# lorenzrichter/path-space-PDE-solver

Hardware: AMD Instinct MI355X
Metric: trajectory-timesteps/sec (K*N/s), d=100 HJB log-variance training iteration (higher is better)
Workload: dtype f32 (f16x3 split products: every matrix product as three f16 MFMAs, fp32 accumulate; state / sums fp32)

## Files before the change

### path-space-pde-solver_amd/csrc/hjb_kernels.h

```cpp
#pragma once
#include <cstdlib>
#include <type_traits>
#include <hip/hip_runtime.h>
#include <stdint.h>

namespace psp {

typedef float f32x4 __attribute__((ext_vector_type(4)));

struct HjbArgs {
    const float* params;
    const float* x0;
    const float* y0;
    const float* xi;
    float* path;
    float* D;
    float* XN;
    double* fwd_partial;
    const float* drift;
    const float* sigma;
    const float* runcost;
    const float* term;
    const double* sums;
    float* grad_partial;
// ... 95 lines not shown
    return p + opaque_i(0);
}

#define PSP_PATH_STORE(ptr, val) __builtin_nontemporal_store((val), (ptr))

#ifndef PSP_PHILOX_ROUNDS
#define PSP_PHILOX_ROUNDS 7
#endif
constexpr int kPhiloxRounds = PSP_PHILOX_ROUNDS;
__device__ __forceinline__ void philox4x32_R(uint32_t c0, uint32_t c1, uint32_t c2, uint32_t c3,
                                             uint32_t k0, uint32_t k1, uint32_t (&out)[4]) {
#pragma unroll
    for (int r = 0; r < kPhiloxRounds; ++r) {
        const unsigned long long p0 = (unsigned long long)0xD2511F53u * (unsigned long long)c0;
        const unsigned long long p1 = (unsigned long long)0xCD9E8D57u * (unsigned long long)c2;
        const uint32_t hi0 = (uint32_t)(p0 >> 32), lo0 = (uint32_t)p0;
        const uint32_t hi1 = (uint32_t)(p1 >> 32), lo1 = (uint32_t)p1;
        const uint32_t n0 = __builtin_amdgcn_bitop3_b32(hi1, c1, k0, 0x96), n2 = __builtin_amdgcn_bitop3_b32(hi0, c3, k1, 0x96);
        c0 = n0; c1 = lo1; c2 = n2; c3 = lo0;
        k0 += 0x9E3779B9u; k1 += 0xBB67AE85u;
    }
    out[0] = c0; out[1] = c1; out[2] = c2; out[3] = c3;
}

__device__ __forceinline__ void philox_round(uint32_t& c0, uint32_t& c1, uint32_t& c2, uint32_t& c3, uint32_t k0, uint32_t k1) {
    const unsigned long long p0 = (unsigned long long)0xD2511F53u * (unsigned long long)c0;
    const unsigned long long p1 = (unsigned long long)0xCD9E8D57u * (unsigned long long)c2;
    const uint32_t hi0 = (uint32_t)(p0 >> 32), lo0 = (uint32_t)p0;
    const uint32_t hi1 = (uint32_t)(p1 >> 32), lo1 = (uint32_t)p1;
    const uint32_t n0 = __builtin_amdgcn_bitop3_b32(hi1, c1, k0, 0x96), n2 = __builtin_amdgcn_bitop3_b32(hi0, c3, k1, 0x96);
    c0 = n0; c1 = lo1; c2 = n2; c3 = lo0;
}

__device__ __forceinline__ f32x4 normal4(const uint32_t (&r)[4]) {
    const float s24 = 1.0f / 16777216.0f, h24 = 0.5f / 16777216.0f;
    const float u0 = __builtin_fmaf((float)(r[0] >> 8), s24, h24);
    const float u1 = __builtin_fmaf((float)(r[1] >> 8), s24, h24);
    const float u2 = __builtin_fmaf((float)(r[2] >> 8), s24, h24);
    const float u3 = __builtin_fmaf((float)(r[3] >> 8), s24, h24);
    const float ra = __builtin_amdgcn_sqrtf(-1.3862943611198906f * __builtin_amdgcn_logf(u0));
    const float rb = __builtin_amdgcn_sqrtf(-1.3862943611198906f * __builtin_amdgcn_logf(u2));
    f32x4 z;
    z[0] = ra * __builtin_amdgcn_cosf(u1);
    z[1] = ra * __builtin_amdgcn_sinf(u1);
    z[2] = rb * __builtin_amdgcn_cosf(u3);
    z[3] = rb * __builtin_amdgcn_sinf(u3);
    return z;
}

__device__ __forceinline__ f32x4 philox_block(uint32_t kglob, uint32_t step, uint32_t idx, uint32_t iter,
                                              uint32_t seed_lo, uint32_t seed_hi) {
    uint32_t r[4];
    philox4x32_R(kglob, step, idx, iter, seed_lo, seed_hi, r);
    return normal4(r);
}

template <int D, int DB>
__device__ __forceinline__ void regen_xi(f32x4 (&xin)[DB], uint32_t kglob, uint32_t n, int q, uint32_t iter,
                                         uint32_t seed_lo, uint32_t seed_hi) {
#pragma unroll
    for (int b = 0; b < DB; ++b) {
        xin[b] = philox_block(kglob, n, (uint32_t)(4 * b + q), iter, seed_lo, seed_hi);
        if (16 * b + 16 > D) {
#pragma unroll
            for (int r = 0; r < 4; ++r) if (16 * b + 4 * r + q >= D) xin[b][r] = 0.f;
        }
    }
}

template <class F>
__device__ __forceinline__ void stage_aop(float* dst, int MB, int KS, int tid, int nthr, F src) {
    const int total = MB * KS * 64;
    for (int idx = tid; idx < total; idx += nthr) {
        const int lane = idx & 63, t = idx >> 6;
        const int ks = t % KS, mb = t / KS;
        const int i = lane & 15, q = lane >> 4;
        dst[idx] = src(16 * mb + 4 * (i & 3) + (i >> 2), 4 * ks + q);
    }
}
template <class F>
__device__ __forceinline__ void stage_vec(float* dst, int NBLK, int tid, int nthr, F v) {
    for (int idx = tid; idx < NBLK * 16; idx += nthr) {
        const int r = idx & 3, q = (idx >> 2) & 3, b = idx >> 4;
        dst[idx] = v(16 * b + 4 * r + q);
    }
}
// ... 456 lines not shown
    __syncthreads();

    const int t16 = blockIdx.x * nwave + wave;
    const bool wave_valid = t16 < a.ntile16;
    const int k = t16 * 16 + j;
    const bool kvalid = wave_valid && k < a.K_local;
    const uint32_t kglob = (uint32_t)(a.k_offset + k);
    const float dt = a.dt, sqdt = a.sqdt;

    const float store_cxi = SPEC ? 1.f : ((k_store == 3) ? 0.f : 1.f);
    const float store_cz = SPEC ? 0.f : ((k_store == 3) ? 1.f : (k_store == 2 ? -a.sqdt : (k_adaptive ? 0.f : a.sqdt)));
    const bool do_store = FAST ? true : (k_store != 0);
    double sD = 0.0, sD2 = 0.0;
    if (wave_valid) {
        const f32x4* vecs0 = reinterpret_cast<const f32x4*>(lds + VEC) + q;
        const f32x4* vterm = vecs0 + (G::vterm - G::fVec) / 4;

        f32x4 X[DB];
#pragma unroll
        for (int b = 0; b < DB; ++b) {
#pragma unroll
            for (int r = 0; r < 4; ++r) {
                const int f = 16 * b + 4 * r + q;
                const float v = a.x0[(size_t)(kvalid ? k : 0) * a.x0_stride + (f < D ? f : D - 1)];
                X[b][r] = (f < D && kvalid) ? v : 0.f;
            }
        }
        float Y = a.y0 ? a.y0[0] : 0.f;
        float Fsum = 0.f, ULsum = 0.f;
#ifdef PSP_STAMPS
        unsigned long long stamps[8] = {0, 0, 0, 0, 0, 0, 0, 0};
#endif

        for (int n = 0; n < a.N; ++n) {
            PSP_STAMP(fs0);
            float tn = (float)n * dt;
            if constexpr (!FAST) { if (a.tfeat) tn = a.tfeat[n]; }
            const f32x4* vecs = opaque(vecs0);
            const f32x4* vb1 = vecs + (G::vb1 - G::fVec) / 4;
            const f32x4* vw1t = vecs + (G::vw1t - G::fVec) / 4;
            const f32x4* vb2 = vecs + (G::vb2 - G::fVec) / 4;
            const f32x4* vb3 = vecs + (G::vb3 - G::fVec) / 4;
            const f32x4* vdr = vecs + (G::vdr - G::fVec) / 4;
            const f32x4* vrun = vecs + (G::vrun - G::fVec) / 4;
            float* pblk = a.path + ((size_t)n * a.ntile16 + t16) * (size_t)G::PB + lane;
            auto x_store = [&](int u, int NU) __attribute__((always_inline)) {
                if (do_store) {
#pragma unroll
                    for (int ks = 0; ks < 4 * DB; ++ks)
                        if (ks >= u * (4 * DB) / NU && ks < (u + 1) * (4 * DB) / NU)
                            PSP_PATH_STORE(pblk + (G::pX / 64 + ks) * 64, X[ks >> 2][ks & 3]);
                }
            };
            if (!X3 && do_store) {
#pragma unroll
                for (int ks = 0; ks < 4 * DB; ++ks) PSP_PATH_STORE(pblk + (G::pX / 64 + ks) * 64, X[ks >> 2][ks & 3]);
            }
            f32x4 h1[HB];
#pragma unroll
            for (int m = 0; m < HB; ++m) h1[m] = vb1[m * 4] + tn * vw1t[m * 4];
            f32x4 Tn[DB];
            const bool early_drift = X3 && k_drift == DRIFT_DENSE;
            if constexpr (X3) {
                if (k_drift == DRIFT_DENSE) {
                    f16x8 xh[DB / 2 > 0 ? DB / 2 : 1], xl[DB / 2 > 0 ? DB / 2 : 1];
                    constexpr int NU1 = (DB / 2) * HB, NU2 = (DB / 2) * DB;
                    split_panel8<DB>(X, xh, xl);
                    gemm_Txs<HB, KSD, DB, 2>(h1, lds + oW1, xh, xl, X[DB - 1], lane, [&](int u) __attribute__((always_inline)) { x_store(u, NU1 + NU2); });
#pragma unroll
                    for (int b = 0; b < DB; ++b) Tn[b] = X[b];
                    gemm_Txs<DB, KSD, DB, 2>(Tn, ldsA, xh, xl, X[DB - 1], lane, [&](int u) __attribute__((always_inline)) { x_store(NU1 + u, NU1 + NU2); });
                    if constexpr (NU1 + NU2 == 0) x_store(0, 1);
                } else {
                    constexpr int NU1 = (DB / 2) * HB;
                    gemm_Tx<HB, KSD, DB, 2>(h1, lds + oW1, X, lane, [&](int u) __attribute__((always_inline)) { x_store(u, NU1); });
                    if constexpr (NU1 == 0) x_store(0, 1);
                }
            }
            else if constexpr (BF16) gemm_Tb<HB, DB>(h1, lds + oW1, X, lane);
            else gemm_T<HB, KSD, DB>(h1, lds + oW1, X, lane);
            PSP_STAMP(fs1);
#pragma unroll
            for (int m = 0; m < HB; ++m) h1[m] = tanh4(h1[m]);
            PSP_STAMP(fs2);
            f32x4 h2[HB];
#pragma unroll
            for (int m = 0; m < HB; ++m) h2[m] = vb2[m * 4];
            constexpr int NUH2 = (HB / 2) * HB, NUH3 = (HB / 2) * DB;
            constexpr bool PREGEN = X3 && FAST && (NUH2 + NUH3 > 0);
            [[maybe_unused]] f32x4 xig[PREGEN ? DB : 1];
            [[maybe_unused]] uint32_t pc0 = 0, pc1 = 0, pc2 = 0, pc3 = 0;
            constexpr int NSPC = kPhiloxRounds + 1;
            auto philox_slice = [&](int sidx) __attribute__((always_inline)) {
                const int b = sidx / NSPC, sub = sidx % NSPC;
                if (sub == 0) { pc0 = kglob; pc1 = (uint32_t)n; pc2 = (uint32_t)(4 * b + q); pc3 = iter_now; }
                if (sub < kPhiloxRounds) {
                    philox_round(pc0, pc1, pc2, pc3, a.seed_lo + (uint32_t)sub * 0x9E3779B9u, a.seed_hi + (uint32_t)sub * 0xBB67AE85u);
                    asm volatile("" : "+v"(pc0), "+v"(pc1), "+v"(pc2), "+v"(pc3));
                } else {
                    const uint32_t rr[4] = {pc0, pc1, pc2, pc3};
                    f32x4 xi = normal4(rr);
                    if (16 * b + 16 > D) {
#pragma unroll
                        for (int r = 0; r < 4; ++r) if (16 * b + 4 * r + q >= D) xi[r] = 0.f;
                    }
                    asm volatile("" : "+v"(xi));
                    xig[b < DB ? b : 0] = xi;
                }
            };
            auto philox_portion = [&](int u) __attribute__((always_inline)) {
                if constexpr (PREGEN) {
#pragma unroll
                    for (int sidx = 0; sidx < NSPC * DB; ++sidx)
                        if (sidx >= u * (NSPC * DB) / (NUH2 + NUH3) && sidx < (u + 1) * (NSPC * DB) / (NUH2 + NUH3)) philox_slice(sidx);
                }
            };
            auto h_store = [&](const f32x4 (&h)[HB], int slot, int u, int NU) __attribute__((always_inline)) {
                if (do_store) {
#pragma unroll
                    for (int ks = 0; ks < 4 * HB; ++ks)
                        if (ks >= u * (4 * HB) / NU && ks < (u + 1) * (4 * HB) / NU)
                            PSP_PATH_STORE(pblk + (slot / 64 + ks) * 64, h[ks >> 2][ks & 3]);
                }
            };
            if constexpr (X3) {
                gemm_Tx<HB, KSH, HB, 2>(h2, lds + oW2, h1, lane, [&](int u) __attribute__((always_inline)) { h_store(h1, G::pH1, u, NUH2); philox_portion(u); });
                if constexpr (NUH2 == 0) h_store(h1, G::pH1, 0, 1);
            }
            else if constexpr (BF16) gemm_Tb<HB, HB>(h2, lds + oW2, h1, lane);
            else gemm_T<HB, KSH, HB>(h2, lds + oW2, h1, lane);
// ... 615 lines not shown
```

### path-space-pde-solver_amd/csrc/hjbx_kernels.h

```cpp
#pragma once
#include "hjb_kernels.h"

namespace psp {

template <int D, int H>
struct GeoX {
    using G = Geo<D, H>;
    static constexpr int DB = G::DB, HB = G::HB, KSD = G::KSD, KSH = G::KSH;
    static constexpr int T3 = 0, T2 = T3 + SplitGeo<KSD, DB>::floats(HB), EX = T2 + SplitGeo<KSH, HB>::floats(HB);
    static constexpr int hG = 0, hGl = hG + D * 32, hZ2 = hGl + D * 32, hZ2l = hZ2 + HB * 512, hZ1 = hZ2l + HB * 512,
                         hZ1l = hZ1 + HB * 512, PAIRH = hZ1l + HB * 512;
    static constexpr int RS = 16 * DB + 3 * 16 * HB;
    static constexpr int NX = cdiv(DB, 4);
    static constexpr int NT = DB + 2 * HB;
    static_assert(4 * RS <= 4 * (PAIRH / 2), "bias sums reuse the exchange area");
    static constexpr int GS = EX + 4 * (PAIRH / 2);
    static int lds_floats() { return GS + 12; }
};

template <int NB>
__device__ __forceinline__ void split_panel(const f32x4 (&v)[NB], f16x4 (&hi)[NB], f16x4 (&lo)[NB]) {
#pragma unroll
    for (int b = 0; b < NB; ++b) {
        if ((NB & 1) && b == NB - 1) split4c(v[b], hi[b], lo[b]);
        else split4(v[b], hi[b], lo[b]);
    }
}

template <int MB, int KS, int INB>
__device__ __forceinline__ void gemm_Txp(f32x4 (&acc)[MB], const float* wlds, const f16x4 (&hi)[INB], const f16x4 (&lo)[INB],
                                         float last, int lane) {
    using SG = SplitGeo<KS, INB>;
    constexpr int NS = SG::NS;
    lane = opaque_i(lane);
    f32x4 corr[MB];
#pragma unroll
    for (int mb = 0; mb < MB; ++mb) corr[mb] = f32x4{0.f, 0.f, 0.f, 0.f};
    if constexpr (NS > 0) {
        const f16x8* tbl = reinterpret_cast<const f16x8*>(wlds) + lane;
        constexpr int NU = NS * MB, CU = 1, NCH = cdiv(NU, CU);
        f16x8 ah[2][CU], al[2][CU];
#pragma unroll
        for (int kk = 0; kk < CU; ++kk)
            if (kk < NU) {
                ah[0][kk] = tbl[((kk % MB) * SG::per_mb + (kk / MB) * 512) / 4];
                al[0][kk] = tbl[((kk % MB) * SG::per_mb + (kk / MB) * 512) / 4 + 64];
            }
#pragma unroll
// ... 17 lines not shown
                    const f16x8 bl = __builtin_shufflevector(lo[2 * S], lo[2 * S + 1], 0, 1, 2, 3, 4, 5, 6, 7);
                    acc[mb] = __builtin_amdgcn_mfma_f32_16x16x32_f16(ah[c & 1][kk], bh, acc[mb], 0, 0, 0);
                    corr[mb] = __builtin_amdgcn_mfma_f32_16x16x32_f16(ah[c & 1][kk], bl, corr[mb], 0, 0, 0);
                    corr[mb] = __builtin_amdgcn_mfma_f32_16x16x32_f16(al[c & 1][kk], bh, corr[mb], 0, 0, 0);
                }
            }
            __builtin_amdgcn_sched_barrier(kFenceMask);
        }
    }
    if constexpr (SG::ODD_F32) {
#pragma unroll
        for (int mb = 0; mb < MB; ++mb) acc[mb] = mfma16(wlds[mb * SG::per_mb + NS * 512 + lane], last, acc[mb]);
    }
    if constexpr (SG::ODD_H16) {
#pragma unroll
        for (int mb = 0; mb < MB; ++mb) {
            const f16x4* p = reinterpret_cast<const f16x4*>(wlds + mb * SG::per_mb + NS * 512) + lane;
            const f16x4 a_hi = p[0], a_lo = p[64];
            acc[mb] = __builtin_amdgcn_mfma_f32_16x16x16f16(a_hi, hi[INB - 1], acc[mb], 0, 0, 0);
            corr[mb] = __builtin_amdgcn_mfma_f32_16x16x16f16(a_hi, lo[INB - 1], corr[mb], 0, 0, 0);
            corr[mb] = __builtin_amdgcn_mfma_f32_16x16x16f16(a_lo, hi[INB - 1], corr[mb], 0, 0, 0);
        }
    }
#pragma unroll
    for (int mb = 0; mb < MB; ++mb) acc[mb] = acc[mb] + kSplitInv * corr[mb];
}

template <int D, int H, bool REGEN = false>
__global__ __launch_bounds__(512) void hjb_bwd3_kernel(const HjbArgs a) {
    PSP_COND_EXIT(a);
    GradCheck<true> gchk;
    using G = Geo<D, H>;
    using X = GeoX<D, H>;
    constexpr int DB = G::DB, HB = G::HB, KSD = G::KSD, KSH = G::KSH, NX = X::NX, RS = X::RS, PAIRH = X::PAIRH, NT = X::NT;
    extern __shared__ __attribute__((aligned(16))) float lds[];
    const int tid = threadIdx.x, nthr = blockDim.x;
    const int lane = tid & 63, wave = __builtin_amdgcn_readfirstlane(tid >> 6);
    const int j = lane & 15, q = lane >> 4;
    const bool producer = wave < 4;
    const int sub = wave & 3;
    const float* __restrict__ P = a.params;

    const double invK = 1.0 / (double)a.K_global;
    const float meanD = (a.loss_kind == LOSS_LOGVAR) ? (float)(a.sums[0] * invK) : 0.f;
    const float coef = (float)(2.0 * invK);
    {
        float wm = 0.f;
        for (int k = tid; k < a.K_local; k += nthr) {
            const float dk = a.D[k];
            wm = fmaxf(wm, fabsf(a.loss_kind == LOSS_WEIGHTS ? dk : coef * (dk - meanD)));
        }
#pragma unroll
        for (int o = 1; o < 64; o <<= 1) wm = fmaxf(wm, __shfl_xor(wm, o));
        if (lane == 0) lds[X::GS + 4 + wave] = wm;
    }
    stage_aop_x3<KSD, DB>(lds + X::T3, HB, tid, nthr, [&](int row, int col) {
        return (row < H && col < D) ? P[G::oW3 + col * H + row] : 0.f; });
    stage_aop_x3<KSH, HB>(lds + X::T2, HB, tid, nthr, [&](int row, int col) {
        return (row < H && col < H) ? P[G::oW2 + col * H + row] : 0.f; });
    __syncthreads();
    _Float16* exh = reinterpret_cast<_Float16*>(lds + X::EX);
    const bool xi_image = a.adaptive != 0 && (a.store_path == 1 || a.store_path == 4);
    auto g_scale = [&](float& gs, float& ginv) __attribute__((always_inline)) {
        const float* slot = lds + X::GS;
        float imax = fmaxf(fmaxf(slot[0], slot[1]), fmaxf(slot[2], slot[3]));
        if (xi_image || !(imax >= 1.1754944e-38f)) imax = xi_image ? 8.0f : 1.0f;
        const float wmax = fmaxf(fmaxf(fmaxf(slot[4], slot[5]), fmaxf(slot[6], slot[7])),
                                 fmaxf(fmaxf(slot[8], slot[9]), fmaxf(slot[10], slot[11])));
        const float amax = wmax * a.sqdt * imax;
        const unsigned e = (__float_as_uint(amax) >> 23) & 0xFFu;
        const bool ok = e >= 1u && e <= 253u;
        gs = ok ? __uint_as_float((254u - e) << 23) : 1.0f;
        ginv = ok ? __uint_as_float(e << 23) : 1.0f;
    };
    const f32x4 zero4 = {0.f, 0.f, 0.f, 0.f};
    const float sqdt = a.sqdt, dt = a.dt;
    constexpr bool regen = REGEN;
    const uint32_t iter_now = a.iter_dev ? *a.iter_dev : a.iter;
    const long long nblk = (long long)a.N * a.ntile16;
    const long long nround = (nblk + 3) / 4;
    const int R = (int)((nround - blockIdx.x + gridDim.x - 1) / gridDim.x);

    if (producer) {
        f32x4 sG[DB], sZ2[HB], sZ1[HB], sT1[HB];
#pragma unroll
        for (int b = 0; b < DB; ++b) sG[b] = zero4;
#pragma unroll
        for (int m = 0; m < HB; ++m) { sZ2[m] = zero4; sZ1[m] = zero4; sT1[m] = zero4; }
        auto own_block = [&](int it2) __attribute__((always_inline)) {
            const long long b0 = ((long long)blockIdx.x + (long long)it2 * gridDim.x) * 4 + sub;
            return b0 < nblk ? b0 : -1LL;
        };
        auto path_of = [&](int it2) __attribute__((always_inline)) {
            const long long b0 = own_block(it2);
            return a.path + (size_t)(b0 >= 0 ? b0 : nblk - 1) * (size_t)G::PB + lane;
        };
        f32x4 xin[DB], h2n[HB], h1n[HB];
        float dkn;
        {
            const long long b0 = own_block(0);
            const long long blk = b0 >= 0 ? b0 : nblk - 1;
            const float* pb = path_of(0);
            const int k0 = (int)(blk % a.ntile16) * 16 + j;
            dkn = a.D[k0 < a.K_local ? k0 : 0];
            if constexpr (regen) {
#pragma unroll
                for (int b = 0; b < DB; ++b) xin[b] = zero4;
            } else {
#pragma unroll
                for (int b = 0; b < DB; ++b)
#pragma unroll
                    for (int r = 0; r < 4; ++r) xin[b][r] = pb[G::pXi + (4 * b + r) * 64];
            }
            if constexpr (regen) {
#pragma unroll
                for (int m = 0; m < HB; ++m)
#pragma unroll
                    for (int r = 0; r < 4; ++r) h2n[m][r] = pb[G::pH2 + (4 * m + r) * 64];
#pragma unroll
                for (int m = 0; m < HB; ++m)
#pragma unroll
                    for (int r = 0; r < 4; ++r) h1n[m][r] = pb[G::pH1 + (4 * m + r) * 64];
            }
        }
        float gs, ginv;
        {
            const long long b0 = own_block(0);
            const int k0 = (int)((b0 >= 0 ? b0 : nblk - 1) % a.ntile16) * 16 + j;
            const bool kv = b0 >= 0 && k0 < a.K_local;
            float am = 0.f;
#pragma unroll
            for (int b = 0; b < DB; ++b)
#pragma unroll
                for (int r = 0; r < 4; ++r) am = fmaxf(am, kv ? fabsf(xin[b][r]) : 0.f);
#pragma unroll
            for (int o = 1; o < 64; o <<= 1) am = fmaxf(am, __shfl_xor(am, o));
            if (lane == 0) lds[X::GS + sub] = am;
            __syncthreads();
            g_scale(gs, ginv);
        }
#ifdef PSP_STAMPS
        unsigned long long stamps[8] = {0, 0, 0, 0, 0, 0, 0, 0};
#endif
        for (int it = 0; it <= R; ++it) {
            PSP_STAMP(tp0);
            if (it < R) {
                const long long blk0 = own_block(it);
                const bool bvalid = blk0 >= 0;
                const long long blk = bvalid ? blk0 : nblk - 1;
                const int t16 = (int)(blk % a.ntile16);
                const int k = t16 * 16 + j;
                const bool kvalid = bvalid && k < a.K_local;
                const float tn = (float)(blk / a.ntile16) * dt;
                _Float16* ex0 = exh + ((it & 1) * 2 + (sub >> 1)) * PAIRH + (sub & 1) * 4 + (j & 3);
                _Float16* exr[4] = {ex0 + (((j >> 2) ^ 0) * 8), ex0 + (((j >> 2) ^ 1) * 8), ex0 + (((j >> 2) ^ 2) * 8), ex0 + (((j >> 2) ^ 3) * 8)};
                const float* pn = path_of(it + 1);
                const float* pc = path_of(it);
                const float dkc = dkn;
                if constexpr (!regen) {
#pragma unroll
                    for (int m = 0; m < HB; ++m)
#pragma unroll
                        for (int r = 0; r < 4; ++r) h2n[m][r] = pc[G::pH2 + (4 * m + r) * 64];
                }
                const float wk = kvalid ? (a.loss_kind == LOSS_WEIGHTS ? dkc : coef * (dkc - meanD)) : 0.f;
                f32x4 Gt[DB];
                if constexpr (regen) {
                    const uint32_t kg = (uint32_t)(a.k_offset + k), nstep = (uint32_t)(blk / a.ntile16);
                    const int qo = opaque_i(q);
#pragma unroll
                    for (int b = 0; b < DB; ++b) {
                        f32x4 xi = philox_block(kg, nstep, (uint32_t)(4 * b + qo), iter_now, a.seed_lo, a.seed_hi);
                        if (16 * b + 16 > D) {
#pragma unroll
                            for (int r = 0; r < 4; ++r) if (16 * b + 4 * r + q >= D) xi[r] = 0.f;
                        }
                        {
#pragma clang fp contract(off)
                            Gt[b] = (wk * sqdt * gs) * xi;
                            sG[b] += Gt[b];
                        }
                        __builtin_amdgcn_sched_barrier(0);
                    }
                } else {
                    {
#pragma clang fp contract(off)
#pragma unroll
                        for (int b = 0; b < DB; ++b) {
                            Gt[b] = (wk * sqdt * gs) * xin[b];
                            sG[b] += Gt[b];
                        }
                    }
                }
                PSP_STAMP(tp1);
                PSP_ACC(0, tp1, tp0);
                f16x4 Gh[DB], Gl[DB];
                split_panel<DB>(Gt, Gh, Gl);
#pragma unroll
                for (int b = 0; b < DB; ++b)
#pragma unroll
                    for (int r = 0; r < 4; ++r) {
                        const int f = 16 * b + 4 * r + q;
                        if (16 * b + 16 <= D || f < D) {
                            exr[r][X::hG + f * 32] = Gh[b][r];
                            exr[r][X::hGl + f * 32] = Gl[b][r];
                        }
                    }
                PSP_STAMP(tp2);
                PSP_ACC(1, tp2, tp1);
                f32x4 dz2[HB];
#pragma unroll
                for (int m = 0; m < HB; ++m) dz2[m] = zero4;
                gemm_Txp<HB, KSD, DB>(dz2, lds + X::T3, Gh, Gl, Gt[DB - 1][0], lane);
                {
#pragma clang fp contract(off)
#pragma unroll
                    for (int m = 0; m < HB; ++m) { dz2[m] = dz2[m] * (1.0f - h2n[m] * h2n[m]); sZ2[m] += dz2[m]; }
                }
                if constexpr (regen) {
                    __builtin_amdgcn_sched_barrier(0);
#pragma unroll
                    for (int m = 0; m < HB; ++m)
#pragma unroll
                        for (int r = 0; r < 4; ++r) h2n[m][r] = pn[G::pH2 + (4 * m + r) * 64];
                } else {
#pragma unroll
                    for (int m = 0; m < HB; ++m)
#pragma unroll
                        for (int r = 0; r < 4; ++r) h1n[m][r] = pc[G::pH1 + (4 * m + r) * 64];
                    const long long n0 = own_block(it + 1);
                    const long long nb1 = n0 >= 0 ? n0 : nblk - 1;
                    const int k1 = (int)(nb1 % a.ntile16) * 16 + j;
                    dkn = a.D[k1 < a.K_local ? k1 : 0];
#pragma unroll
                    for (int b = 0; b < DB; ++b)
#pragma unroll
                        for (int r = 0; r < 4; ++r) xin[b][r] = pn[G::pXi + (4 * b + r) * 64];
                }
                PSP_STAMP(tp3);
                PSP_ACC(2, tp3, tp2);
                f16x4 Zh[HB], Zl[HB];
                split_panel<HB>(dz2, Zh, Zl);
#pragma unroll
                for (int m = 0; m < HB; ++m)
#pragma unroll
                    for (int r = 0; r < 4; ++r) {
                        exr[r][X::hZ2 + (16 * m + 4 * r + q) * 32] = Zh[m][r];
                        exr[r][X::hZ2l + (16 * m + 4 * r + q) * 32] = Zl[m][r];
                    }
                f32x4 dz1[HB];
#pragma unroll
                for (int m = 0; m < HB; ++m) dz1[m] = zero4;
                gemm_Txp<HB, KSH, HB>(dz1, lds + X::T2, Zh, Zl, dz2[HB - 1][0], lane);
                {
#pragma clang fp contract(off)
#pragma unroll
                    for (int m = 0; m < HB; ++m) {
                        dz1[m] = dz1[m] * (1.0f - h1n[m] * h1n[m]);
                        sZ1[m] += dz1[m];
                        sT1[m] += tn * dz1[m];
                    }
                }
                if constexpr (regen) {
                    __builtin_amdgcn_sched_barrier(0);
                    const long long n0 = own_block(it + 1);
                    const long long nb1 = n0 >= 0 ? n0 : nblk - 1;
                    const int k1 = (int)(nb1 % a.ntile16) * 16 + j;
                    dkn = a.D[k1 < a.K_local ? k1 : 0];
#pragma unroll
                    for (int m = 0; m < HB; ++m)
#pragma unroll
                        for (int r = 0; r < 4; ++r) h1n[m][r] = pn[G::pH1 + (4 * m + r) * 64];
                }
                split_panel<HB>(dz1, Zh, Zl);
#pragma unroll
                for (int m = 0; m < HB; ++m)
#pragma unroll
                    for (int r = 0; r < 4; ++r) {
                        exr[r][X::hZ1 + (16 * m + 4 * r + q) * 32] = Zh[m][r];
                        exr[r][X::hZ1l + (16 * m + 4 * r + q) * 32] = Zl[m][r];
                    }
            }
            PSP_STAMP(tp4);
            PSP_ACC(3, tp4, tp0);
            __syncthreads();
            PSP_STAMP(tp5);
            PSP_ACC(4, tp5, tp4);
            PSP_ACC(6, tp5, tp0);
        }
#ifdef PSP_STAMPS
        if (a.dbg && lane == 0) {
            stamps[7] = (unsigned long long)R;
            for (int i = 0; i < 8; ++i) a.dbg[((size_t)blockIdx.x * 8 + wave) * 8 + i] = stamps[i];
        }
#endif
        float* red = lds + X::EX + sub * RS;
#pragma unroll
        for (int b = 0; b < DB; ++b)
#pragma unroll
            for (int r = 0; r < 4; ++r) {
                const float v = ginv * jsumf(sG[b][r]);
                if (j == 0) red[16 * b + 4 * r + q] = v;
            }
#pragma unroll
        for (int m = 0; m < HB; ++m)
#pragma unroll
            for (int r = 0; r < 4; ++r) {
                const float v2 = ginv * jsumf(sZ2[m][r]), v1 = ginv * jsumf(sZ1[m][r]), vt = ginv * jsumf(sT1[m][r]);
                if (j == 0) {
                    red[16 * DB + 16 * m + 4 * r + q] = v2;
                    red[16 * DB + 16 * HB + 16 * m + 4 * r + q] = v1;
                    red[16 * DB + 32 * HB + 16 * m + 4 * r + q] = vt;
                }
            }
        __syncthreads();
        return;
    }
    const int ibw = sub < HB ? sub : HB - 1;
    int obx[NX];
#pragma unroll
    for (int s = 0; s < NX; ++s) obx[s] = (sub + 4 * s) < DB ? (sub + 4 * s) : DB - 1;
    f32x4 a3[DB], a2[HB], a1[HB][NX], c1[HB][NX];
#pragma unroll
    for (int b = 0; b < DB; ++b) a3[b] = zero4;
#pragma unroll
    for (int m = 0; m < HB; ++m) {
        a2[m] = zero4;
#pragma unroll
        for (int s = 0; s < NX; ++s) { a1[m][s] = zero4; c1[m][s] = zero4; }
    }
    const int nblk_i = (int)nblk;
    auto blk_at = [&](long long c0) __attribute__((always_inline)) {
        const int c = (c0 < (long long)nblk_i) ? (int)c0 : nblk_i - 1;
        return __builtin_amdgcn_readfirstlane(c);
    };
    typedef const __attribute__((address_space(1))) float* gptr_t;
    auto sbase = [&](int blk, int ofs) __attribute__((always_inline)) {
        return (gptr_t)sgpr_block_addr(a.path, (unsigned long long)blk, (unsigned)G::PB, (unsigned)ofs);
    };
    const unsigned lofsU = (unsigned)image_lane_offset_F(lane);
    auto get_F = [&](gptr_t base) __attribute__((always_inline)) {
        return *reinterpret_cast<const __attribute__((address_space(1))) f32x4*>(base + lofsU);
    };
    f32x4 Lh2[2], Lh1[2], Lx[NX][2];
    auto issue = [&](int c0, int c1) __attribute__((always_inline)) {
        Lh2[0] = get_F(sbase(c0, G::pH2 + ibw * 256)); Lh2[1] = get_F(sbase(c1, G::pH2 + ibw * 256));
        Lh1[0] = get_F(sbase(c0, G::pH1 + ibw * 256)); Lh1[1] = get_F(sbase(c1, G::pH1 + ibw * 256));
#pragma unroll
        for (int s = 0; s < NX; ++s) {
            Lx[s][0] = get_F(sbase(c0, G::pX + obx[s] * 256));
            Lx[s][1] = get_F(sbase(c1, G::pX + obx[s] * 256));
        }
    };
    auto pack = [&](const f32x4& u0, const f32x4& u1, f16x8& hi, f16x8& lo) __attribute__((always_inline)) {
        split8(u0, u1, hi, lo);
    };
    const int aofs = opaque_i((lane & 15) * 32 + (((lane >> 4) ^ ((lane >> 2) & 3)) * 8));
    auto a_load = [&](const _Float16* e, int t, f16x8& Ah, f16x8& Al) __attribute__((always_inline)) {
        const int hi = t < DB ? X::hG + t * 512 : (t < DB + HB ? X::hZ2 + (t - DB) * 512 : X::hZ1 + (t - DB - HB) * 512);
        const int lo = t < DB ? X::hGl + t * 512 : (t < DB + HB ? X::hZ2l + (t - DB) * 512 : X::hZ1l + (t - DB - HB) * 512);
        Ah = *reinterpret_cast<const f16x8*>(e + hi + aofs);
        Al = *reinterpret_cast<const f16x8*>(e + lo + aofs);
    };
    const f16x8 k2048 = {(_Float16)2048.f, (_Float16)2048.f, (_Float16)2048.f, (_Float16)2048.f,
                         (_Float16)2048.f, (_Float16)2048.f, (_Float16)2048.f, (_Float16)2048.f};
    auto pair_phase = [&](const _Float16* e, int n0, int n1) __attribute__((always_inline)) {
        f16x8 Ah[3], Al[3];
        a_load(e, 0, Ah[0], Al[0]);
        a_load(e, 1, Ah[1], Al[1]);
        f16x8 h2h, h2l, h1h, h1l, xh[NX], xl[NX];
        pack(Lh2[0], Lh2[1], h2h, h2l);
        pack(Lh1[0], Lh1[1], h1h, h1l);
#pragma unroll
        for (int s = 0; s < NX; ++s) pack(Lx[s][0], Lx[s][1], xh[s], xl[s]);
        const f16x8 h2s = h2h * k2048, h1s = h1h * k2048;
        __builtin_amdgcn_sched_barrier(0);
        issue(n0, n1);
        __builtin_amdgcn_sched_barrier(0);
#pragma unroll
        for (int t = 0; t < NT; ++t) {
            if (t + 2 < NT) a_load(e, t + 2, Ah[(t + 2) % 3], Al[(t + 2) % 3]);
            const f16x8 ah = Ah[t % 3], al = Al[t % 3];
            if (t < DB) {
                a3[t] = __builtin_amdgcn_mfma_f32_16x16x32_f16(ah, h2s, a3[t], 0, 0, 0);
                a3[t] = __builtin_amdgcn_mfma_f32_16x16x32_f16(ah, h2l, a3[t], 0, 0, 0);
                a3[t] = __builtin_amdgcn_mfma_f32_16x16x32_f16(al, h2h, a3[t], 0, 0, 0);
            } else if (t < DB + HB) {
                const int m = t - DB;
                a2[m] = __builtin_amdgcn_mfma_f32_16x16x32_f16(ah, h1s, a2[m], 0, 0, 0);
                a2[m] = __builtin_amdgcn_mfma_f32_16x16x32_f16(ah, h1l, a2[m], 0, 0, 0);
                a2[m] = __builtin_amdgcn_mfma_f32_16x16x32_f16(al, h1h, a2[m], 0, 0, 0);
            } else {
                const int m = t - DB - HB;
#pragma unroll
                for (int s = 0; s < NX; ++s) {
                    a1[m][s] = __builtin_amdgcn_mfma_f32_16x16x32_f16(ah, xh[s], a1[m][s], 0, 0, 0);
                    c1[m][s] = __builtin_amdgcn_mfma_f32_16x16x32_f16(ah, xl[s], c1[m][s], 0, 0, 0);
                    c1[m][s] = __builtin_amdgcn_mfma_f32_16x16x32_f16(al, xh[s], c1[m][s], 0, 0, 0);
                }
            }
            __builtin_amdgcn_sched_barrier(kFenceMask);
        }
    };

    {
        const long long rb = (long long)blockIdx.x * 4;
        issue(blk_at(rb), blk_at(rb + 1));
    }
    __syncthreads();
    __syncthreads();
#ifdef PSP_STAMPS
    unsigned long long stamps[8] = {0, 0, 0, 0, 0, 0, 0, 0};
#endif
    for (int it = 1; it <= R; ++it) {
        PSP_STAMP(tc0);
        const long long rb = ((long long)blockIdx.x + (long long)(it - 1) * gridDim.x) * 4;
        const _Float16* exr = exh + ((it - 1) & 1) * 2 * PAIRH;
        const long long rn = rb + 4LL * gridDim.x;
        pair_phase(exr, blk_at(rb + 2), blk_at(rb + 3));
        PSP_STAMP(tc1);
        pair_phase(exr + PAIRH, blk_at(rn), blk_at(rn + 1));
        PSP_STAMP(tc2);
        PSP_ACC(0, tc2, tc0);
        PSP_ACC(1, tc1, tc0);
        __syncthreads();
        PSP_STAMP(tc3);
        PSP_ACC(4, tc3, tc2);
        PSP_ACC(6, tc3, tc0);
    }
#ifdef PSP_STAMPS
    if (a.dbg && lane == 0) {
        stamps[7] = (unsigned long long)R;
        for (int i = 0; i < 8; ++i) a.dbg[((size_t)blockIdx.x * 8 + wave) * 8 + i] = stamps[i];
    }
#endif
    float gs, ginv;
    g_scale(gs, ginv);
    const float inv1 = ginv, inv2 = ginv * kSplitInv;

    float* gp = a.grad_partial + (size_t)blockIdx.x * G::P;
    const int col = lane & 15, qq = lane >> 4;
    if (sub < HB) {
#pragma unroll
        for (int b = 0; b < DB; ++b) {
            const f32x4 v = inv2 * a3[b];
#pragma unroll
            for (int rr = 0; rr < 4; ++rr) {
                const int o3 = 16 * b + 4 * qq + rr, i3 = 16 * sub + col;
                if (o3 < D && i3 < H) { const float gv_ = v[rr]; gp[G::oW3 + o3 * H + i3] = gv_; gchk.see(gv_); }
            }
        }
#pragma unroll
        for (int m = 0; m < HB; ++m) {
            const f32x4 v = inv2 * a2[m];
#pragma unroll
            for (int rr = 0; rr < 4; ++rr) {
                const int o2 = 16 * m + 4 * qq + rr, i2 = 16 * sub + col;
                if (o2 < H && i2 < H) { const float gv_ = v[rr]; gp[G::oW2 + o2 * H + i2] = gv_; gchk.see(gv_); }
            }
        }
    }
#pragma unroll
    for (int m = 0; m < HB; ++m)
#pragma unroll
        for (int s = 0; s < NX; ++s) {
            const f32x4 v = inv1 * (a1[m][s] + kSplitInv * c1[m][s]);
            const int ob = sub + 4 * s;
#pragma unroll
            for (int rr = 0; rr < 4; ++rr) {
                const int o1 = 16 * m + 4 * qq + rr, i1 = 16 * ob + col;
                if (ob < DB && o1 < H && i1 < D) { const float gv_ = v[rr]; gp[G::oW1 + o1 * (D + 1) + 1 + i1] = gv_; gchk.see(gv_); }
            }
        }
    __syncthreads();
    {
        const float* red = lds + X::EX;
        const int ct = tid - 256;
        for (int f = ct; f < D; f += 256)
            { const float gv_ = (red[f] + red[RS + f]) + (red[2 * RS + f] + red[3 * RS + f]); gp[G::ob3 + f] = gv_; gchk.see(gv_); }
        for (int f = ct; f < H; f += 256) {
            const float* r2 = red + 16 * DB + f;
            { const float gv_ = (r2[0] + r2[RS]) + (r2[2 * RS] + r2[3 * RS]); gp[G::ob2 + f] = gv_; gchk.see(gv_); }
            const float* r1 = r2 + 16 * HB;
            { const float gv_ = (r1[0] + r1[RS]) + (r1[2 * RS] + r1[3 * RS]); gp[G::ob1 + f] = gv_; gchk.see(gv_); }
            const float* rt = r1 + 16 * HB;
            { const float gv_ = (rt[0] + rt[RS]) + (rt[2 * RS] + rt[3 * RS]); gp[G::oW1 + f * (D + 1)] = gv_; gchk.see(gv_); }
        }
    }
    gchk.raise(a.cond);
}

template <int D, int H>
struct HjbxLaunch {
    using X = GeoX<D, H>;
    static int lds_bytes() { return X::lds_floats() * 4; }
    static hipError_t bwd(const HjbArgs& a, int grid, hipStream_t s) {
        const int bytes = lds_bytes();
        if (a.store_path == 4) {
            hipError_t e = hipFuncSetAttribute(reinterpret_cast<const void*>(&hjb_bwd3_kernel<D, H, true>),
                                               hipFuncAttributeMaxDynamicSharedMemorySize, bytes);
            if (e != hipSuccess) return e;
            hipLaunchKernelGGL((hjb_bwd3_kernel<D, H, true>), dim3(grid), dim3(512), bytes, s, a);
            return hipGetLastError();
        }
        hipError_t e = hipFuncSetAttribute(reinterpret_cast<const void*>(&hjb_bwd3_kernel<D, H, false>),
                                           hipFuncAttributeMaxDynamicSharedMemorySize, bytes);
        if (e != hipSuccess) return e;
        hipLaunchKernelGGL((hjb_bwd3_kernel<D, H, false>), dim3(grid), dim3(512), bytes, s, a);
        return hipGetLastError();
    }
};

}
```

Measured before the change: 1.640 billion.

## Move bias-gradient sums into MFMA consumer pass and precompute Philox prefix rounds

```diff
diff --git a/path-space-pde-solver_amd/csrc/hjb_kernels.h b/path-space-pde-solver_amd/csrc/hjb_kernels.h
--- a/path-space-pde-solver_amd/csrc/hjb_kernels.h
+++ b/path-space-pde-solver_amd/csrc/hjb_kernels.h
@@ -151,6 +151,28 @@
     c0 = n0; c1 = lo1; c2 = n2; c3 = lo0;
 }
 
+struct PhiloxPrefix { uint32_t lo0, hi1, lo1; };
+constexpr unsigned long long kPhiloxIdxStep = 4ull * 0xCD9E8D57ull;
+__device__ __forceinline__ PhiloxPrefix philox_prefix(uint32_t kglob, uint32_t iter, uint32_t k1) {
+    const unsigned long long p0 = (unsigned long long)0xD2511F53u * (unsigned long long)kglob;
+    const uint32_t n2 = __builtin_amdgcn_bitop3_b32((uint32_t)(p0 >> 32), iter, k1, 0x96);
+    const unsigned long long p1 = (unsigned long long)0xCD9E8D57u * (unsigned long long)n2;
+    return PhiloxPrefix{(uint32_t)p0, (uint32_t)(p1 >> 32), (uint32_t)p1};
+}
+__device__ __forceinline__ unsigned long long philox_idx_base(int q) {
+    return (unsigned long long)0xCD9E8D57u * (unsigned long long)(uint32_t)q;
+}
+__device__ __forceinline__ void philox_head(const PhiloxPrefix& pf, unsigned long long idx_prod, uint32_t step, uint32_t k0, uint32_t k1,
+                                            uint32_t& c0, uint32_t& c1, uint32_t& c2, uint32_t& c3) {
+    static_assert(kPhiloxRounds >= 2, "the two-stage form covers the first two rounds");
+    const uint32_t n0 = __builtin_amdgcn_bitop3_b32((uint32_t)(idx_prod >> 32), step, k0, 0x96);
+    const unsigned long long p0 = (unsigned long long)0xD2511F53u * (unsigned long long)n0;
+    c0 = __builtin_amdgcn_bitop3_b32(pf.hi1, (uint32_t)idx_prod, k0 + 0x9E3779B9u, 0x96);
+    c1 = pf.lo1;
+    c2 = __builtin_amdgcn_bitop3_b32((uint32_t)(p0 >> 32), pf.lo0, k1 + 0xBB67AE85u, 0x96);
+    c3 = (uint32_t)p0;
+}
+
 __device__ __forceinline__ f32x4 normal4(const uint32_t (&r)[4]) {
     const float s24 = 1.0f / 16777216.0f, h24 = 0.5f / 16777216.0f;
     const float u0 = __builtin_fmaf((float)(r[0] >> 8), s24, h24);
@@ -171,6 +193,15 @@
                                               uint32_t seed_lo, uint32_t seed_hi) {
     uint32_t r[4];
     philox4x32_R(kglob, step, idx, iter, seed_lo, seed_hi, r);
+    return normal4(r);
+}
+__device__ __forceinline__ f32x4 philox_block_pf(const PhiloxPrefix& pf, unsigned long long idx_prod, uint32_t step,
+                                                 uint32_t seed_lo, uint32_t seed_hi) {
+    uint32_t r[4];
+    philox_head(pf, idx_prod, step, seed_lo, seed_hi, r[0], r[1], r[2], r[3]);
+#pragma unroll
+    for (int i = 2; i < kPhiloxRounds; ++i)
+        philox_round(r[0], r[1], r[2], r[3], seed_lo + (uint32_t)i * 0x9E3779B9u, seed_hi + (uint32_t)i * 0xBB67AE85u);
     return normal4(r);
 }
 
@@ -693,6 +724,8 @@
         unsigned long long stamps[8] = {0, 0, 0, 0, 0, 0, 0, 0};
 #endif
 
+        [[maybe_unused]] const PhiloxPrefix ppf = philox_prefix(kglob, iter_now, a.seed_hi);
+        [[maybe_unused]] const unsigned long long pidx0 = philox_idx_base(q);
         for (int n = 0; n < a.N; ++n) {
             PSP_STAMP(fs0);
             float tn = (float)n * dt;
@@ -751,12 +784,14 @@
             constexpr bool PREGEN = X3 && FAST && (NUH2 + NUH3 > 0);
             [[maybe_unused]] f32x4 xig[PREGEN ? DB : 1];
             [[maybe_unused]] uint32_t pc0 = 0, pc1 = 0, pc2 = 0, pc3 = 0;
-            constexpr int NSPC = kPhiloxRounds + 1;
+            constexpr int NSPC = kPhiloxRounds;
             auto philox_slice = [&](int sidx) __attribute__((always_inline)) {
                 const int b = sidx / NSPC, sub = sidx % NSPC;
-                if (sub == 0) { pc0 = kglob; pc1 = (uint32_t)n; pc2 = (uint32_t)(4 * b + q); pc3 = iter_now; }
-                if (sub < kPhiloxRounds) {
-                    philox_round(pc0, pc1, pc2, pc3, a.seed_lo + (uint32_t)sub * 0x9E3779B9u, a.seed_hi + (uint32_t)sub * 0xBB67AE85u);
+                if (sub == 0) {
+                    philox_head(ppf, pidx0 + (unsigned long long)b * kPhiloxIdxStep, (uint32_t)n, a.seed_lo, a.seed_hi, pc0, pc1, pc2, pc3);
+                    asm volatile("" : "+v"(pc0), "+v"(pc1), "+v"(pc2), "+v"(pc3));
+                } else if (sub < NSPC - 1) {
+                    philox_round(pc0, pc1, pc2, pc3, a.seed_lo + (uint32_t)(sub + 1) * 0x9E3779B9u, a.seed_hi + (uint32_t)(sub + 1) * 0xBB67AE85u);
                     asm volatile("" : "+v"(pc0), "+v"(pc1), "+v"(pc2), "+v"(pc3));
                 } else {
                     const uint32_t rr[4] = {pc0, pc1, pc2, pc3};
diff --git a/path-space-pde-solver_amd/csrc/hjbx_kernels.h b/path-space-pde-solver_amd/csrc/hjbx_kernels.h
--- a/path-space-pde-solver_amd/csrc/hjbx_kernels.h
+++ b/path-space-pde-solver_amd/csrc/hjbx_kernels.h
@@ -10,10 +10,8 @@
     static constexpr int T3 = 0, T2 = T3 + SplitGeo<KSD, DB>::floats(HB), EX = T2 + SplitGeo<KSH, HB>::floats(HB);
     static constexpr int hG = 0, hGl = hG + D * 32, hZ2 = hGl + D * 32, hZ2l = hZ2 + HB * 512, hZ1 = hZ2l + HB * 512,
                          hZ1l = hZ1 + HB * 512, PAIRH = hZ1l + HB * 512;
-    static constexpr int RS = 16 * DB + 3 * 16 * HB;
     static constexpr int NX = cdiv(DB, 4);
     static constexpr int NT = DB + 2 * HB;
-    static_assert(4 * RS <= 4 * (PAIRH / 2), "bias sums reuse the exchange area");
     static constexpr int GS = EX + 4 * (PAIRH / 2);
     static int lds_floats() { return GS + 12; }
 };
@@ -97,7 +95,7 @@
     GradCheck<true> gchk;
     using G = Geo<D, H>;
     using X = GeoX<D, H>;
-    constexpr int DB = G::DB, HB = G::HB, KSD = G::KSD, KSH = G::KSH, NX = X::NX, RS = X::RS, PAIRH = X::PAIRH, NT = X::NT;
+    constexpr int DB = G::DB, HB = G::HB, KSD = G::KSD, KSH = G::KSH, NX = X::NX, PAIRH = X::PAIRH, NT = X::NT;
     extern __shared__ __attribute__((aligned(16))) float lds[];
     const int tid = threadIdx.x, nthr = blockDim.x;
     const int lane = tid & 63, wave = __builtin_amdgcn_readfirstlane(tid >> 6);
@@ -147,26 +145,23 @@
     const int R = (int)((nround - blockIdx.x + gridDim.x - 1) / gridDim.x);
 
     if (producer) {
-        f32x4 sG[DB], sZ2[HB], sZ1[HB], sT1[HB];
-#pragma unroll
-        for (int b = 0; b < DB; ++b) sG[b] = zero4;
-#pragma unroll
-        for (int m = 0; m < HB; ++m) { sZ2[m] = zero4; sZ1[m] = zero4; sT1[m] = zero4; }
-        auto own_block = [&](int it2) __attribute__((always_inline)) {
-            const long long b0 = ((long long)blockIdx.x + (long long)it2 * gridDim.x) * 4 + sub;
-            return b0 < nblk ? b0 : -1LL;
+        const int bstep = 4 * (int)gridDim.x, adv_n = bstep / a.ntile16, adv_t = bstep % a.ntile16;
+        int bn, bt;
+        {
+            const unsigned b0 = blockIdx.x * 4u + (unsigned)sub;
+            bn = (int)(b0 / (unsigned)a.ntile16); bt = (int)(b0 % (unsigned)a.ntile16);
+        }
+        auto path_at = [&](int n, int t16) __attribute__((always_inline)) {
+            const bool v = n < a.N;
+            return a.path + ((size_t)(v ? n : a.N - 1) * (size_t)a.ntile16 + (size_t)(v ? t16 : a.ntile16 - 1)) * (size_t)G::PB + lane;
         };
-        auto path_of = [&](int it2) __attribute__((always_inline)) {
-            const long long b0 = own_block(it2);
-            return a.path + (size_t)(b0 >= 0 ? b0 : nblk - 1) * (size_t)G::PB + lane;
-        };
+        auto tile_at = [&](int n, int t16) __attribute__((always_inline)) { return n < a.N ? t16 : a.ntile16 - 1; };
         f32x4 xin[DB], h2n[HB], h1n[HB];
         float dkn;
+        [[maybe_unused]] const unsigned long long idx_base = philox_idx_base(q);
         {
-            const long long b0 = own_block(0);
-            const long long blk = b0 >= 0 ? b0 : nblk - 1;
-            const float* pb = path_of(0);
-            const int k0 = (int)(blk % a.ntile16) * 16 + j;
+            const float* pb = path_at(bn, bt);
+            const int k0 = tile_at(bn, bt) * 16 + j;
             dkn = a.D[k0 < a.K_local ? k0 : 0];
             if constexpr (regen) {
 #pragma unroll
@@ -190,9 +185,8 @@
         }
         float gs, ginv;
         {
-            const long long b0 = own_block(0);
-            const int k0 = (int)((b0 >= 0 ? b0 : nblk - 1) % a.ntile16) * 16 + j;
-            const bool kv = b0 >= 0 && k0 < a.K_local;
+            const int k0 = tile_at(bn, bt) * 16 + j;
+            const bool kv = bn < a.N && k0 < a.K_local;
             float am = 0.f;
 #pragma unroll
             for (int b = 0; b < DB; ++b)
@@ -210,17 +204,16 @@
         for (int it = 0; it <= R; ++it) {
             PSP_STAMP(tp0);
             if (it < R) {
-                const long long blk0 = own_block(it);
-                const bool bvalid = blk0 >= 0;
-                const long long blk = bvalid ? blk0 : nblk - 1;
-                const int t16 = (int)(blk % a.ntile16);
+                const bool bvalid = bn < a.N;
+                const int nstep_i = bvalid ? bn : a.N - 1, t16 = tile_at(bn, bt);
+                int nn = bn + adv_n, nt = bt + adv_t;
+                if (nt >= a.ntile16) { nt -= a.ntile16; ++nn; }
                 const int k = t16 * 16 + j;
                 const bool kvalid = bvalid && k < a.K_local;
-                const float tn = (float)(blk / a.ntile16) * dt;
                 _Float16* ex0 = exh + ((it & 1) * 2 + (sub >> 1)) * PAIRH + (sub & 1) * 4 + (j & 3);
                 _Float16* exr[4] = {ex0 + (((j >> 2) ^ 0) * 8), ex0 + (((j >> 2) ^ 1) * 8), ex0 + (((j >> 2) ^ 2) * 8), ex0 + (((j >> 2) ^ 3) * 8)};
-                const float* pn = path_of(it + 1);
-                const float* pc = path_of(it);
+                const float* pn = path_at(nn, nt);
+                const float* pc = path_at(bn, bt);
                 const float dkc = dkn;
                 if constexpr (!regen) {
 #pragma unroll
@@ -231,31 +224,24 @@
                 const float wk = kvalid ? (a.loss_kind == LOSS_WEIGHTS ? dkc : coef * (dkc - meanD)) : 0.f;
                 f32x4 Gt[DB];
                 if constexpr (regen) {
-                    const uint32_t kg = (uint32_t)(a.k_offset + k), nstep = (uint32_t)(blk / a.ntile16);
-                    const int qo = opaque_i(q);
+                    const uint32_t kg = (uint32_t)(a.k_offset + k), nstep = (uint32_t)nstep_i;
+                    const PhiloxPrefix pf = philox_prefix(kg, iter_now, a.seed_hi);
+                    uint32_t ib_lo = (uint32_t)idx_base, ib_hi = (uint32_t)(idx_base >> 32);
+                    asm volatile("" : "+v"(ib_lo), "+v"(ib_hi));
+                    const unsigned long long ib = ((unsigned long long)ib_hi << 32) | ib_lo;
 #pragma unroll
                     for (int b = 0; b < DB; ++b) {
-                        f32x4 xi = philox_block(kg, nstep, (uint32_t)(4 * b + qo), iter_now, a.seed_lo, a.seed_hi);
+                        f32x4 xi = philox_block_pf(pf, ib + (unsigned long long)b * kPhiloxIdxStep, nstep, a.seed_lo, a.seed_hi);
                         if (16 * b + 16 > D) {
 #pragma unroll
                             for (int r = 0; r < 4; ++r) if (16 * b + 4 * r + q >= D) xi[r] = 0.f;
                         }
-                        {
-#pragma clang fp contract(off)
-                            Gt[b] = (wk * sqdt * gs) * xi;
-                            sG[b] += Gt[b];
-                        }
+                        Gt[b] = (wk * sqdt * gs) * xi;
                         __builtin_amdgcn_sched_barrier(0);
                     }
                 } else {
-                    {
-#pragma clang fp contract(off)
-#pragma unroll
-                        for (int b = 0; b < DB; ++b) {
-                            Gt[b] = (wk * sqdt * gs) * xin[b];
-                            sG[b] += Gt[b];
-                        }
-                    }
+#pragma unroll
+                    for (int b = 0; b < DB; ++b) Gt[b] = (wk * sqdt * gs) * xin[b];
                 }
                 PSP_STAMP(tp1);
                 PSP_ACC(0, tp1, tp0);
@@ -280,7 +266,7 @@
                 {
 #pragma clang fp contract(off)
 #pragma unroll
-                    for (int m = 0; m < HB; ++m) { dz2[m] = dz2[m] * (1.0f - h2n[m] * h2n[m]); sZ2[m] += dz2[m]; }
+                    for (int m = 0; m < HB; ++m) dz2[m] = dz2[m] * (1.0f - h2n[m] * h2n[m]);
                 }
                 if constexpr (regen) {
                     __builtin_amdgcn_sched_barrier(0);
@@ -293,9 +279,7 @@
                     for (int m = 0; m < HB; ++m)
 #pragma unroll
                         for (int r = 0; r < 4; ++r) h1n[m][r] = pc[G::pH1 + (4 * m + r) * 64];
-                    const long long n0 = own_block(it + 1);
-                    const long long nb1 = n0 >= 0 ? n0 : nblk - 1;
-                    const int k1 = (int)(nb1 % a.ntile16) * 16 + j;
+                    const int k1 = tile_at(nn, nt) * 16 + j;
                     dkn = a.D[k1 < a.K_local ? k1 : 0];
 #pragma unroll
                     for (int b = 0; b < DB; ++b)
@@ -320,17 +304,11 @@
                 {
 #pragma clang fp contract(off)
 #pragma unroll
-                    for (int m = 0; m < HB; ++m) {
-                        dz1[m] = dz1[m] * (1.0f - h1n[m] * h1n[m]);
-                        sZ1[m] += dz1[m];
-                        sT1[m] += tn * dz1[m];
-                    }
+                    for (int m = 0; m < HB; ++m) dz1[m] = dz1[m] * (1.0f - h1n[m] * h1n[m]);
                 }
                 if constexpr (regen) {
                     __builtin_amdgcn_sched_barrier(0);
-                    const long long n0 = own_block(it + 1);
-                    const long long nb1 = n0 >= 0 ? n0 : nblk - 1;
-                    const int k1 = (int)(nb1 % a.ntile16) * 16 + j;
+                    const int k1 = tile_at(nn, nt) * 16 + j;
                     dkn = a.D[k1 < a.K_local ? k1 : 0];
 #pragma unroll
                     for (int m = 0; m < HB; ++m)
@@ -345,6 +323,7 @@
                         exr[r][X::hZ1 + (16 * m + 4 * r + q) * 32] = Zh[m][r];
                         exr[r][X::hZ1l + (16 * m + 4 * r + q) * 32] = Zl[m][r];
                     }
+                bn = nn; bt = nt;
             }
             PSP_STAMP(tp4);
             PSP_ACC(3, tp4, tp0);
@@ -359,26 +338,6 @@
             for (int i = 0; i < 8; ++i) a.dbg[((size_t)blockIdx.x * 8 + wave) * 8 + i] = stamps[i];
         }
 #endif
-        float* red = lds + X::EX + sub * RS;
-#pragma unroll
-        for (int b = 0; b < DB; ++b)
-#pragma unroll
-            for (int r = 0; r < 4; ++r) {
-                const float v = ginv * jsumf(sG[b][r]);
-                if (j == 0) red[16 * b + 4 * r + q] = v;
-            }
-#pragma unroll
-        for (int m = 0; m < HB; ++m)
-#pragma unroll
-            for (int r = 0; r < 4; ++r) {
-                const float v2 = ginv * jsumf(sZ2[m][r]), v1 = ginv * jsumf(sZ1[m][r]), vt = ginv * jsumf(sT1[m][r]);
-                if (j == 0) {
-                    red[16 * DB + 16 * m + 4 * r + q] = v2;
-                    red[16 * DB + 16 * HB + 16 * m + 4 * r + q] = v1;
-                    red[16 * DB + 32 * HB + 16 * m + 4 * r + q] = vt;
-                }
-            }
-        __syncthreads();
         return;
     }
     const int ibw = sub < HB ? sub : HB - 1;
@@ -394,6 +353,33 @@
 #pragma unroll
         for (int s = 0; s < NX; ++s) { a1[m][s] = zero4; c1[m][s] = zero4; }
     }
+    constexpr int NBT = cdiv(NT, 4);
+    f32x4 sB[NBT];
+#pragma unroll
+    for (int i = 0; i < NBT; ++i) sB[i] = zero4;
+    const int bcol = lane & 15;
+    auto bias_ops = [&](float t0, float t1, f16x8& B1, f16x8& B2) __attribute__((always_inline)) {
+        _Float16 th0, tl0, th1, tl1;
+        split_f16(t0, th0, tl0);
+        split_f16(t1, th1, tl1);
+        const _Float16 one = (_Float16)1.f, nil = (_Float16)0.f;
+        const _Float16 p0 = bcol == 0 ? one : (bcol == 1 ? th0 : (bcol == 2 ? tl0 : nil)), p1 = bcol == 0 ? one : (bcol == 1 ? th1 : (bcol == 2 ? tl1 : nil));
+        const _Float16 s0 = bcol == 2 ? th0 : (bcol == 3 ? one : nil), s1 = bcol == 2 ? th1 : (bcol == 3 ? one : nil);
+        B1 = f16x8{p0, p0, p0, p0, p1, p1, p1, p1};
+        B2 = f16x8{s0, s0, s0, s0, s1, s1, s1, s1};
+    };
+    const int bstep = 4 * (int)gridDim.x, adv_n = bstep / a.ntile16, adv_t = bstep % a.ntile16;
+    int rn, rt;
+    {
+        const unsigned b0 = blockIdx.x * 4u;
+        rn = (int)(b0 / (unsigned)a.ntile16); rt = (int)(b0 % (unsigned)a.ntile16);
+    }
+    auto time_of = [&](int i) __attribute__((always_inline)) {
+        int n = rn, t = rt + i;
+#pragma unroll
+        for (int c = 0; c < 3; ++c) if (t >= a.ntile16) { t -= a.ntile16; ++n; }
+        return (float)(n < a.N ? n : a.N - 1) * dt;
+    };
     const int nblk_i = (int)nblk;
     auto blk_at = [&](long long c0) __attribute__((always_inline)) {
         const int c = (c0 < (long long)nblk_i) ? (int)c0 : nblk_i - 1;
@@ -429,8 +415,9 @@
     };
     const f16x8 k2048 = {(_Float16)2048.f, (_Float16)2048.f, (_Float16)2048.f, (_Float16)2048.f,
                          (_Float16)2048.f, (_Float16)2048.f, (_Float16)2048.f, (_Float16)2048.f};
-    auto pair_phase = [&](const _Float16* e, int n0, int n1) __attribute__((always_inline)) {
-        f16x8 Ah[3], Al[3];
+    auto pair_phase = [&](const _Float16* e, int n0, int n1, float t0, float t1) __attribute__((always_inline)) {
+        f16x8 Ah[3], Al[3], B1, B2;
+        bias_ops(t0, t1, B1, B2);
         a_load(e, 0, Ah[0], Al[0]);
         a_load(e, 1, Ah[1], Al[1]);
         f16x8 h2h, h2l, h1h, h1l, xh[NX], xl[NX];
@@ -446,6 +433,10 @@
         for (int t = 0; t < NT; ++t) {
             if (t + 2 < NT) a_load(e, t + 2, Ah[(t + 2) % 3], Al[(t + 2) % 3]);
             const f16x8 ah = Ah[t % 3], al = Al[t % 3];
+            if ((t & 3) == sub) {
+                sB[t >> 2] = __builtin_amdgcn_mfma_f32_16x16x32_f16(ah, B1, sB[t >> 2], 0, 0, 0);
+                sB[t >> 2] = __builtin_amdgcn_mfma_f32_16x16x32_f16(al, B2, sB[t >> 2], 0, 0, 0);
+            }
             if (t < DB) {
                 a3[t] = __builtin_amdgcn_mfma_f32_16x16x32_f16(ah, h2s, a3[t], 0, 0, 0);
                 a3[t] = __builtin_amdgcn_mfma_f32_16x16x32_f16(ah, h2l, a3[t], 0, 0, 0);
@@ -481,10 +472,12 @@
         PSP_STAMP(tc0);
         const long long rb = ((long long)blockIdx.x + (long long)(it - 1) * gridDim.x) * 4;
         const _Float16* exr = exh + ((it - 1) & 1) * 2 * PAIRH;
-        const long long rn = rb + 4LL * gridDim.x;
-        pair_phase(exr, blk_at(rb + 2), blk_at(rb + 3));
+        const long long rnx = rb + 4LL * gridDim.x;
+        pair_phase(exr, blk_at(rb + 2), blk_at(rb + 3), time_of(0), time_of(1));
         PSP_STAMP(tc1);
-        pair_phase(exr + PAIRH, blk_at(rn), blk_at(rn + 1));
+        pair_phase(exr + PAIRH, blk_at(rnx), blk_at(rnx + 1), time_of(2), time_of(3));
+        rn += adv_n; rt += adv_t;
+        if (rt >= a.ntile16) { rt -= a.ntile16; ++rn; }
         PSP_STAMP(tc2);
         PSP_ACC(0, tc2, tc0);
         PSP_ACC(1, tc1, tc0);
@@ -537,19 +530,25 @@
                 if (ob < DB && o1 < H && i1 < D) { const float gv_ = v[rr]; gp[G::oW1 + o1 * (D + 1) + 1 + i1] = gv_; gchk.see(gv_); }
             }
         }
-    __syncthreads();
-    {
-        const float* red = lds + X::EX;
-        const int ct = tid - 256;
-        for (int f = ct; f < D; f += 256)
-            { const float gv_ = (red[f] + red[RS + f]) + (red[2 * RS + f] + red[3 * RS + f]); gp[G::ob3 + f] = gv_; gchk.see(gv_); }
-        for (int f = ct; f < H; f += 256) {
-            const float* r2 = red + 16 * DB + f;
-            { const float gv_ = (r2[0] + r2[RS]) + (r2[2 * RS] + r2[3 * RS]); gp[G::ob2 + f] = gv_; gchk.see(gv_); }
-            const float* r1 = r2 + 16 * HB;
-            { const float gv_ = (r1[0] + r1[RS]) + (r1[2 * RS] + r1[3 * RS]); gp[G::ob1 + f] = gv_; gchk.see(gv_); }
-            const float* rt = r1 + 16 * HB;
-            { const float gv_ = (rt[0] + rt[RS]) + (rt[2 * RS] + rt[3 * RS]); gp[G::oW1 + f * (D + 1)] = gv_; gchk.see(gv_); }
+#pragma unroll
+    for (int i = 0; i < NBT; ++i) {
+        const int t = sub + 4 * i;
+        const f32x4 other = {__shfl(sB[i][0], lane + (col == 0 ? 3 : 1)), __shfl(sB[i][1], lane + (col == 0 ? 3 : 1)),
+                             __shfl(sB[i][2], lane + (col == 0 ? 3 : 1)), __shfl(sB[i][3], lane + (col == 0 ? 3 : 1))};
+        const f32x4 v = inv1 * (sB[i] + kSplitInv * other);
+        if (t < NT && col < 2) {
+#pragma unroll
+            for (int rr = 0; rr < 4; ++rr) {
+                const int f = 16 * (t < DB ? t : (t < DB + HB ? t - DB : t - DB - HB)) + 4 * qq + rr;
+                const float gv_ = v[rr];
+                if (t < DB) {
+                    if (col == 0 && f < D) { gp[G::ob3 + f] = gv_; gchk.see(gv_); }
+                } else if (t < DB + HB) {
+                    if (col == 0 && f < H) { gp[G::ob2 + f] = gv_; gchk.see(gv_); }
+                } else if (f < H) {
+                    gp[col == 0 ? G::ob1 + f : G::oW1 + f * (D + 1)] = gv_; gchk.see(gv_);
+                }
+            }
         }
     }
     gchk.raise(a.cond);
```

After: 1.583 billion. 0.965x the previous value.
